# s-will/BiAlign

Hardware: AMD Instinct MI355X
Metric: giga-DP-cells/sec (higher is better)
Workload: dtype int32

## Files before the change

### bialign_amd/csrc/bialign_feed.hpp

```cpp
#pragma once

namespace bialign {

template <int S, int NL, bool LEAN = false, int BLKO = 0>
struct GhostFeed {
  using R_ = Rec<S, NL, LEAN>;
  static constexpr int W = 2 * S + 1, R = 64 / W;
  static constexpr int NP = R_::NCH4 + (R_::TAIL ? 1 : 0);
#ifdef BIALIGN_BLK_OVERRIDE
  static constexpr int BLK = BIALIGN_BLK_OVERRIDE;
#else
  static constexpr int BLK = BLKO ? BLKO : (S <= 1 ? 8 : 4);
#endif
  static constexpr int NPIECE = BLK * W * NP;
  static constexpr bool PIECE_MAJOR = S >= 2;
  __host__ __device__ static constexpr int slot(int t, int aa, int c) {
    return PIECE_MAJOR ? (c * BLK + t) * W + aa : (t * W + aa) * NP + c;
  }
  static constexpr int ROUNDS = (NPIECE + 63) / 64;
  static constexpr int SLOTS = ROUNDS * 64;
  static constexpr int RING_DW = 2 * SLOTS * 4;
  static constexpr int MIN_GOFF = 2 * BLK + 8;

  __device__ static __forceinline__ void issue(const int32_t* lay, int h0, int blk_q, int blk_rem,
                                               int P, int T, int w, int GOFF, int rec_last, int lane,
                                               uint32_t lds_base) {
#pragma unroll
    for (int r = 0; r < ROUNDS; ++r) {
      const int q = min(r * 64 + lane, NPIECE - 1);
      int t, aa, c;
      if (PIECE_MAJOR) {
        c = q / (BLK * W);
        const int rem = q - c * (BLK * W);
        t = rem / W;
        aa = rem - t * W;
      } else {
        t = q / (W * NP);
        const int rem = q - t * (W * NP);
        aa = rem / NP;
        c = rem - aa * NP;
      }
      const int xr = blk_rem + t - aa;
      const int ql = blk_q + (xr >= P ? 1 : 0) - (xr < 0 ? 1 : 0);
      const int rec = min(max(h0 + t - GOFF + (ql * (T - 1) + w) * P, 0), rec_last);
      const int sl = LEAN ? aa : (R - 2) * W + aa;
      const int32_t* p = lay + (int64_t)rec * R_::RECDW +
                         (c < R_::NCH4 ? c * R_::CH + sl * 4 : R_::NCH4 * R_::CH + sl * R_::TAIL);
      const uint32_t dst = lds_base + r * 1024;
      uint32_t keep;
      asm volatile(
          "s_mov_b32 %0, m0\n\ts_mov_b32 m0, %2\n\ts_nop 0\n\t"
          "global_load_lds_dwordx4 %1, off sc1\n\ts_mov_b32 m0, %0"
          : "=&s"(keep)
          : "v"(p), "s"(dst)
          : "memory");
    }
  }
  __host__ __device__ static inline void piece_of(int q, int& t, int& aa, int& c) {
    if (PIECE_MAJOR) {
      c = q / (BLK * W);
      const int rem = q - c * (BLK * W);
      t = rem / W;
      aa = rem - t * W;
    } else {
      t = q / (W * NP);
      const int rem = q - t * (W * NP);
      aa = rem / NP;
      c = rem - aa * NP;
    }
  }
  __host__ __device__ static inline int packed_piece_dw(int c, int sl) {
    using PK = Pack<S>;
    return c < PK::NCH ? c * R_::CH + sl * 4 : (c == PK::NCH && PK::TAILDW ? PK::NCH * R_::CH + sl * PK::TAILDW : sl * 4);
  }
  template <typename Base>
  __host__ __device__ static inline Base packed_src(Base lay, int q, int64_t bnd_off, int blk_q, int blk_rem, int P, int T,
                                                    int w, int m, int rec_last) {
    using PK = Pack<S>;
    int t, aa, c;
    piece_of(q, t, aa, c);
    const int xr = blk_rem + t - aa;
    const int ql = blk_q + (xr >= P ? 1 : 0) - (xr < 0 ? 1 : 0);
    const int jj = xr - (xr >= P ? P : 0) + (xr < 0 ? P : 0);
    const int ts = jj + 2 * (R - 1) + aa;
    const int cs = ts >= P ? ts - P : ts, qs = ql * T + w - 1 + (ts >= P ? 1 : 0);
    const int64_t rec = (int64_t)(ql * T + w - 1) * P + ts;
    const bool valid = rec >= 0 && rec <= rec_last;
    const int sl = (R - 2) * W + aa;
    if (valid && PK::interior(qs, cs, m)) return lay + rec * PK::RECDW + packed_piece_dw(c, sl);
    return lay + bnd_off + (valid ? PK::bidx(qs, cs, P, m) : 0) * R_::RECDW +
           (c < R_::NCH4 ? c * R_::CH + sl * 4 : R_::NCH4 * R_::CH + sl * R_::TAIL);
  }
  __device__ static __forceinline__ void issue_packed(const int32_t* lay, int64_t bnd_off, int m, int h0, int blk_q,
                                                      int blk_rem, int P, int T, int w, int rec_last, int lane,
                                                      uint32_t lds_base) {
#pragma unroll
    for (int r = 0; r < ROUNDS; ++r) {
      const int q = min(r * 64 + lane, NPIECE - 1);
      const int32_t* p = packed_src(lay, q, bnd_off, blk_q, blk_rem, P, T, w, m, rec_last);
      const uint32_t dst = lds_base + r * 1024;
      uint32_t keep;
      asm volatile(
          "s_mov_b32 %0, m0\n\ts_mov_b32 m0, %2\n\ts_nop 0\n\t"
          "global_load_lds_dwordx4 %1, off sc1\n\ts_mov_b32 m0, %0"
          : "=&s"(keep)
          : "v"(p), "s"(dst)
          : "memory");
    }
  }

  __host__ __device__ static inline bool steady(int blk_q, int blk_rem, int P, int T, int w, int m, int rec_last) {
    using PK = Pack<S>;
    const int qs = blk_q * T + w - 1, ts_last = blk_rem + BLK - 1 + 2 * (R - 1);
    return qs >= PK::Q0 && blk_rem >= 3 * S + 1 && ts_last <= m - S && (int64_t)qs * P + ts_last <= rec_last;
  }
  __host__ __device__ static inline int64_t steady_base_dword(int blk_q, int blk_rem, int P, int T, int w) {
    return ((int64_t)(blk_q * T + w - 1) * P + blk_rem + 2 * (R - 1)) * Pack<S>::RECDW;
  }
  __host__ __device__ static inline uint32_t lane_offset(int r, int lane) {
    int t, aa, c;
    piece_of(r * 64 + lane < NPIECE - 1 ? r * 64 + lane : NPIECE - 1, t, aa, c);
    return (uint32_t)(t * Pack<S>::RECDW + packed_piece_dw(c, (R - 2) * W + aa)) * 4u;
  }
  static constexpr int OFFTAB_DW = ROUNDS * 64;
  __device__ static __forceinline__ void issue_steady(const int32_t* lay, int blk_q, int blk_rem, int P, int T, int w,
                                                      const int32_t* offtab, int lane, uint32_t lds_base) {
    const int32_t* base = lay + steady_base_dword(blk_q, blk_rem, P, T, w);
    uint32_t off[ROUNDS];
#pragma unroll
    for (int r = 0; r < ROUNDS; ++r) off[r] = (uint32_t)offtab[r * 64 + lane];
#pragma unroll
    for (int r = 0; r < ROUNDS; ++r) {
      const uint32_t dst = lds_base + r * 1024;
      uint32_t keep;
      asm volatile(
          "s_mov_b32 %0, m0\n\ts_mov_b32 m0, %2\n\ts_nop 0\n\t"
          "global_load_lds_dwordx4 %1, %3 sc1\n\ts_mov_b32 m0, %0"
          : "=&s"(keep)
          : "v"(off[r]), "s"(dst), "s"(base)
          : "memory");
    }
  }
  static constexpr int STORES_PER_STEP = R_::NCH4 + (R_::TAIL ? 1 : 0);

  __device__ static __forceinline__ void wait_block(int younger) {
    if (younger > 40) asm volatile("s_waitcnt vmcnt(40)" ::: "memory");
    else if (younger > 24) asm volatile("s_waitcnt vmcnt(24)" ::: "memory");
    else if (younger > 20) asm volatile("s_waitcnt vmcnt(20)" ::: "memory");
    else if (younger > 16) asm volatile("s_waitcnt vmcnt(16)" ::: "memory");
    else if (younger > 12) asm volatile("s_waitcnt vmcnt(12)" ::: "memory");
    else if (younger > 6) asm volatile("s_waitcnt vmcnt(6)" ::: "memory");
    else if (younger > 3) asm volatile("s_waitcnt vmcnt(3)" ::: "memory");
    else if (younger > 1) asm volatile("s_waitcnt vmcnt(1)" ::: "memory");
    else asm volatile("s_waitcnt vmcnt(0)" ::: "memory");
  }

  template <int NPK>
  __device__ static __forceinline__ void fetch_pieces(int (&out)[4 * NPK], const v4i* half, int t, int aa) {
#pragma unroll
    for (int c = 0; c < NPK; ++c) {
      const v4i v = half[slot(t, aa, c)];
      out[4 * c] = v.x; out[4 * c + 1] = v.y; out[4 * c + 2] = v.z; out[4 * c + 3] = v.w;
    }
  }

  __device__ static __forceinline__ void fetch(int (&out)[R_::ND], const v4i* half, int t, int aa) {
#pragma unroll
    for (int c = 0; c < NP; ++c) {
      const v4i v = half[slot(t, aa, c)];
      if (4 * c + 0 < R_::ND) out[4 * c + 0 < R_::ND ? 4 * c + 0 : 0] = v.x;
      if (4 * c + 1 < R_::ND) out[4 * c + 1 < R_::ND ? 4 * c + 1 : 0] = v.y;
      if (4 * c + 2 < R_::ND) out[4 * c + 2 < R_::ND ? 4 * c + 2 : 0] = v.z;
      if (4 * c + 3 < R_::ND) out[4 * c + 3 < R_::ND ? 4 * c + 3 : 0] = v.w;
    }
  }
};

template <int S, bool LEAN>
struct GhostSrc {
  using GF = GhostFeed<S, 9, LEAN, 0>;
  static constexpr int W = 2 * S + 1, R = 64 / W;
  static constexpr int STEPB = W * GF::NP * 16;
  static constexpr int HALFB = GF::SLOTS * 16;
  __host__ __device__ static inline uint32_t ring_step_byte(int g) {
    return (uint32_t)(((g / GF::BLK) & 1) * HALFB + (g & (GF::BLK - 1)) * STEPB);
  }
  __host__ __device__ static inline uint32_t factor(int lane) { return lane < R * W ? 1u : 0u; }
  __host__ __device__ static inline uint32_t lane_byte(int lane, uint32_t sent) {
    return lane < R * W ? (uint32_t)((lane % W) * GF::NP * 16) : sent;
  }
};

template <int S>
constexpr int slim_offtab_dw() { return GhostFeed<S, 9>::OFFTAB_DW; }

template <int S>
struct Mu2Feed {
  static constexpr int BLK = GhostFeed<S, 9>::BLK;
  static constexpr int RING_DW = 2 * BLK * 64;
  __device__ static __forceinline__ void issue(const int32_t* tab, int n, int m, int P, int jj0,
                                               int strip, int T, int w, int il, int aa,
                                               uint32_t lds_base) {
    constexpr int RR = Geo<S>::RR;
#pragma unroll
    for (int t = 0; t < BLK; ++t) {
      int jf = jj0 + t, q = strip;
      if (jf >= P) { jf -= P; ++q; }
      int l = jf + S;
      if (l > m) { l = jf - P + S; ++q; }
      const int k = (q * T + w) * RR + il - 1 + aa - S;
      const int kc = min(max(k, 1), n), lc = min(max(l, 1), m);
      const int32_t* p = tab + (int64_t)(kc - 1) * m + (lc - 1);
      const uint32_t dst = lds_base + t * 256;
      uint32_t keep;
      asm volatile(
          "s_mov_b32 %0, m0\n\ts_mov_b32 m0, %2\n\ts_nop 0\n\t"
          "global_load_lds_dword %1, off\n\ts_mov_b32 m0, %0"
          : "=&s"(keep)
          : "v"(p), "s"(dst)
          : "memory");
    }
  }
};

template <int S>
struct Mu1Feed {
  static constexpr int BLK = GhostFeed<S, 9>::BLK;
  static constexpr int RING_DW = 2 * BLK * 64;
  __device__ static __forceinline__ void issue(const int32_t* tab, int n, int m, int P, int jj0, int strip,
                                               int T, int w, int il, uint32_t lds_base) {
    constexpr int RR = Geo<S>::RR;
#pragma unroll
    for (int t = 0; t < BLK; ++t) {
      int jf = jj0 + t, q = strip;
      if (jf >= P) { jf -= P; ++q; }
      const int i = (q * T + w) * RR + il - 1;
      const int ic = min(max(i, 1), n), jc = min(max(jf, 1), m);
      const int32_t* p = tab + (int64_t)(ic - 1) * m + (jc - 1);
      const uint32_t dst = lds_base + t * 256;
      uint32_t keep;
      asm volatile(
          "s_mov_b32 %0, m0\n\ts_mov_b32 m0, %2\n\ts_nop 0\n\t"
          "global_load_lds_dword %1, off\n\ts_mov_b32 m0, %0"
          : "=&s"(keep)
          : "v"(p), "s"(dst)
          : "memory");
    }
  }
};

}
```

### bialign_amd/csrc/bialign_fill_slim.hpp

```cpp
#pragma once

namespace bialign {

template <int S, int TW, int PPW, bool LEAN = false>
__global__ void __launch_bounds__(64 * TW * PPW, 3) fill_affine_slim_kernel(const DeviceBatch A) {
  static_assert(S >= 1, "packed records need a band");
  using PK_ = Pack<S>;
  using G_ = Geo<S>;
  using R_ = Rec<S, 9, LEAN>;
  constexpr int W = G_::W, R = G_::R, RR = G_::RR, PADB = G_::PADB;
  constexpr int ND = R_::ND, NCH4 = R_::NCH4, TAIL = R_::TAIL, RECDW = R_::RECDW;
  static_assert(R * W < 64, "lane 63 must be free: it is the sentinel source of the exchange");
  extern __shared__ __align__(16) int32_t smem[];

  constexpr int T = TW;
  constexpr int NW = TW * PPW;
  const int L = threadIdx.x & 63;
  const int wv = NW == 1 ? 0 : __builtin_amdgcn_readfirstlane(threadIdx.x >> 6);
  const int pw = wv / TW, w = wv - pw * TW;
  const int slot = blockIdx.x * PPW + pw;
  const bool have_pair = slot < A.launch_pairs;
  const int pid = A.order[have_pair ? slot : 0];
  const PairDesc pd = A.pairs[pid];
  const int n = pd.n, m = pd.m, P = pd.P;
  const int il = L / W, aa = L - il * W;
  const bool live = L < R * W;
  const bool ghost = (il == 0);
  int ringfed_v = (ghost || !live) ? 1 : 0;
  asm volatile("" : "+v"(ringfed_v));
  const bool ringfed = ringfed_v != 0;
  int storing_v;
  {
    const int pad_idx0 = L < W ? L : (L >= R * W ? W + (L - R * W) : 64);
    storing_v = ((live && (LEAN ? il == R - 1 : !ghost)) || (!LEAN && pad_idx0 < R_::SLP - R_::SL)) ? 1 : 0;
  }
  asm volatile("" : "+v"(storing_v));
  const bool storing = storing_v != 0;
  const int beta = A.beta, gamma = A.gamma, delta = A.delta;
  const int k1 = A.k1, k2 = A.k2;
  const int gD = gamma + delta, gg = 2 * gamma, ggdd = 2 * gamma + 2 * delta, dd = 2 * delta;

  using GF = GhostFeed<S, 9, LEAN, 0>;
  constexpr int PERW = GF::RING_DW;
  constexpr int SENTBLK = 4 * GF::NP;
  v4i* ring = reinterpret_cast<v4i*>(smem + wv * GF::RING_DW);
  int32_t* sentblk = smem + NW * PERW;
  volatile int32_t* prog_lds = smem + NW * PERW + SENTBLK + pw * TW;
  const volatile int32_t* const fit_floor = smem + NW * PERW + SENTBLK + FIT_FLOOR_WORD;
  const volatile int32_t* const col0_floor = smem + NW * PERW + SENTBLK + COL0_FLOOR_WORD;
  int32_t* offtab = smem + NW * PERW + SENTBLK + LDS_PROG_WORDS;
  int32_t* s1 = offtab + slim_offtab_dw<S>();
  int32_t* s2 = s1 + k1 * k1;
  uint8_t* codes = reinterpret_cast<uint8_t*>(s2 + k2 * k2);
  const int npad = code_pad(n), mpad = code_pad(m, PADB);
  uint8_t* sa = codes + (size_t)pw * A.slim_code_bytes;
  uint8_t* ca = sa + npad;
  uint8_t* sb = ca + npad;
  uint8_t* cb = sb + mpad;

  for (int t = threadIdx.x; t < NW * PERW + SENTBLK; t += 64 * NW) smem[t] = SENT;
  if (threadIdx.x < LDS_PROG_WORDS) smem[NW * PERW + SENTBLK + threadIdx.x] = prog_word_init(threadIdx.x, A.fit);
  if (!LEAN)
    for (int t = threadIdx.x; t < GF::OFFTAB_DW; t += 64 * NW) offtab[t] = (int32_t)GF::lane_offset(t >> 6, t & 63);
  for (int t = threadIdx.x; t < k1 * k1; t += 64 * NW) s1[t] = A.s1[t];
  for (int t = threadIdx.x; t < k2 * k2; t += 64 * NW) s2[t] = A.s2[t];
  if (have_pair) {
    const int tt = threadIdx.x - pw * (64 * TW);
    for (int t = tt; t < n; t += 64 * TW) {
      sa[t] = A.seq_a[pd.seq_a + t];
      ca[t] = A.cls_a[pd.seq_a + t];
    }
    for (int t = tt; t < m + 2 * PADB; t += 64 * TW) {
      const int src = t - PADB;
      const bool ok = src >= 0 && src < m;
      sb[t] = ok ? A.seq_b[pd.seq_b + src] : 0;
      cb[t] = ok ? A.cls_b[pd.seq_b + src] : 0;
    }
  }
  __syncthreads();
  if (!have_pair) return;

  const int addrA = ((L - W) & 63) * 4;
  const int addrB = (live && aa < W - 1 ? ((L - W + 1) & 63) : 63) * 4;
  const bool a_first = (aa == 0);
  const int lane_cap = a_first ? SENT : 0x7fffffff;
  int32_t* const lay = A.layers + pd.layer_off;
  const int64_t pk_bnd_off = (int64_t)pd.G * PK_::RECDW;
  const int rec_last = pd.G - 1;
  const int NSw = (pd.NS - w + T - 1) / T;
  const int H = NSw > 0 ? (NSw - 1) * P + m + G_::MAXOFF + 1 : 0;

  int jj = -(2 * il + aa);
  int strip = 0;
  int rec_base = w * P;
  int i = 0, s1row = 0, s2row = 0;
  bool act_row = false;
  auto set_row = [&](int q) {
    i = (q * T + w) * RR + il - 1;
    const int k = i + aa - S;
    act_row = live && i >= 0 && i <= n && k >= 0 && k <= n;
    s1row = (i >= 1 && i <= n) ? sa[i - 1] * k1 : 0;
    s2row = (k >= 1 && k <= n) ? ca[k - 1] * k2 : 0;
  };
  set_row(0);

  int dA1[2][W], dA2[2][W];
  int dAx[2][W];
  int dB[4][W];
  int dC[2][W];
  int selfv[4][W];
  int pubC[W][8];
  int inC[W][8];
  int inA[W][4], inB[W][8];
#pragma unroll
  for (int bb = 0; bb < W; ++bb) {
    dA1[0][bb] = dA1[1][bb] = dA2[0][bb] = dA2[1][bb] = SENT;
    dAx[0][bb] = dAx[1][bb] = dC[0][bb] = dC[1][bb] = SENT;
#pragma unroll
    for (int x = 0; x < 4; ++x) dB[x][bb] = selfv[x][bb] = inA[bb][x] = SENT;
#pragma unroll
    for (int x = 0; x < 8; ++x) pubC[bb][x] = inB[bb][x] = inC[bb][x] = SENT;
  }
  const uint32_t ring_lds = __builtin_amdgcn_readfirstlane(
      (uint32_t)(uintptr_t)(__attribute__((address_space(3))) int32_t*)smem) + wv * GF::RING_DW * 4;

  using SA = StepAddr<S, LEAN>;
  using GS = GhostSrc<S, LEAN>;
  typedef const __attribute__((address_space(3))) int32_t* lds_cptr;
  typedef __attribute__((address_space(1))) char* gbl_ptr;
  typedef __attribute__((address_space(1))) v4i* gbl_v4i;
  typedef __attribute__((address_space(1))) int32_t* gbl_i32;
  uint32_t st_off = SA::chunk_off(L), st_toff = SA::tail_off(L), gs_fac = GS::factor(L);
  uint32_t gs_lane = GS::lane_byte(L, ring_lds + (NW - wv) * GF::RING_DW * 4);
  asm volatile("" : "+v"(st_off), "+v"(st_toff), "+v"(gs_fac), "+v"(gs_lane));
  int s_ph = 0, s_q = 0;
  int s_adv = 0;
  uint32_t ring_u = 0;
  gbl_ptr sbase = nullptr;

  int blk_q = 0, blk_rem = 0;
  int seen_prog = -0x40000000;
  auto wait_partner = [&](int h_last) __attribute__((always_inline)) {
    if (T == 1) return;
    const int src = w == 0 ? T - 1 : w - 1;
    const int need = h_last + 2 * (R - 1) + 1 - (w == 0 ? P : 0);
    if (seen_prog >= need) return;
    for (int spin = 0; (seen_prog = prog_lds[src]) < need; ++spin) {
      if (spin > A.spin_limit) {
        if (L == 0) atomicOr(A.errflag, 1);
        seen_prog = 0x7fffffff;
        break;
      }
      __builtin_amdgcn_s_sleep(16);
    }
  };
  bool blk_steady = false;
  auto prefetch_block = [&](int h0, int half) __attribute__((always_inline)) {
    wait_partner(h0 + GF::BLK - 1);
    if (!LEAN) blk_steady = GF::steady(blk_q, blk_rem, P, T, w, m, rec_last);
    int Lv = L;
    asm volatile("" : "+v"(Lv));
    if (!LEAN && blk_steady)
      GF::issue_steady(lay, blk_q, blk_rem, P, T, w, offtab, Lv, ring_lds + half * GF::SLOTS * 16);
    else if (LEAN) GF::issue(lay, h0, blk_q, blk_rem, P, T, w, P - 2 * (R - 1), rec_last, Lv, ring_lds + half * GF::SLOTS * 16);
    else GF::issue_packed(lay, pk_bnd_off, m, h0, blk_q, blk_rem, P, T, w, rec_last, Lv, ring_lds + half * GF::SLOTS * 16);
    blk_rem += GF::BLK;
    if (blk_rem >= P) { blk_rem -= P; ++blk_q; }
  };
  prefetch_block(0, 0);
  asm volatile("s_waitcnt vmcnt(0)" ::: "memory");
  int vm_younger = 0;
  int pk_all = 0;
  static_assert(LEAN || PK_::check_in_every_gap(GF::BLK),
                "range check: a test must fall into every non-interior stretch between two strips (pk_all is cleared, not kept, once a row leaves the lattice)");

  auto dmov = [](int& dst, int src) __attribute__((always_inline)) { asm("v_mov_b32 %0, %1" : "=v"(dst) : "v"(src)); };
  auto bperm = [](int addr, int v) __attribute__((always_inline)) -> int { return __builtin_amdgcn_ds_bpermute(addr, v); };

  int mu1n = 0, mu2n[W], sbn = 0, cbn = 0;
  auto lookup_mu = [&]() __attribute__((always_inline)) {
    const int jc = min(max(jj, 0), m + 1);
    mu1n = s1[s1row + sb[jc - 1 + PADB]];
#pragma unroll
    for (int bb = 0; bb < W; ++bb) mu2n[bb] = s2[s2row + cb[jc + bb]];
  };
  auto fetch_codes = [&](auto clamp_tag) __attribute__((always_inline)) {
    const int jc1 = decltype(clamp_tag)::value ? min(max(jj + 1, 0), m + 1) : jj + s_adv + 1;
    sbn = sb[jc1 - 1 + PADB];
    cbn = cb[jc1 + W - 1];
  };
  lookup_mu();
  fetch_codes(BoolTag<true>{});
  int fit_best = SENT, fit_j = 0;

  auto step = [&](auto interior_tag, int g) __attribute__((always_inline)) {
    constexpr bool INTERIOR = decltype(interior_tag)::value;
    if (!INTERIOR) {
      jj += s_adv;
      s_adv = 0;
    }
    const int gt = g & (GF::BLK - 1), ghalf = (g / GF::BLK) & 1;
    if (gt == 0) {
      GF::wait_block(vm_younger);
      if (TW > 1 && L == 0) prog_lds[w] = g - GF::BLK;
      if (!LEAN && (g & (PK_::CHECK - 1)) == 0) {
        const bool bad = live && !ghost && (unsigned)pk_all > 0xffffu;
        if (__builtin_amdgcn_ballot_w64(bad) != 0 && L == 0) atomicOr(A.errflag, 2);
        pk_all = 0;
      }
      if (!LEAN) {
        if (L < GF::BLK * W) {
          bool packed = true;
          if (!blk_steady) {
            int ph = s_ph + L / W, qst = s_q * T + w;
            if (ph >= P) { ph -= P; qst += T; }
            const int ts = ph + 2 * (R - 1), over = ts >= P ? 1 : 0;
            packed = PK_::interior(qst - 1 + over, ts - over * P, m);
          }
          if (packed) {
            v4i* pc = ring + ghalf * GF::SLOTS + L * GF::NP;
            int raw[4 * PK_::NPC], dec[4 * GF::NP];
#pragma unroll
            for (int c = 0; c < PK_::NPC; ++c) {
              const v4i v = pc[c];
              raw[4 * c] = v.x; raw[4 * c + 1] = v.y; raw[4 * c + 2] = v.z; raw[4 * c + 3] = v.w;
            }
#pragma unroll
            for (int d = 0; d < 4 * GF::NP; ++d) {
              const int h = PK_::hw(d < ND ? d : 0);
              const unsigned word = (unsigned)raw[d < ND && d != PK_::ANCHOR ? h >> 1 : 0];
              const unsigned e = d == PK_::ANCHOR ? 0x8000u : PK_::offset_of((h & 1) ? word >> 16 : word & 0xffffu, raw[0]);
              const int v = raw[0] + (int)e;
              dec[d] = d >= ND ? 0 : (pack_corner(W, d % 9, d / 9) ? (e == 0xffffu ? NEG : v) : v);
            }
#pragma unroll
            for (int c = 0; c < GF::NP; ++c) {
              v4i v;
              v.x = dec[4 * c]; v.y = dec[4 * c + 1]; v.z = dec[4 * c + 2]; v.w = dec[4 * c + 3];
              pc[c] = v;
            }
          }
        }
      }
      prefetch_block(g + GF::BLK, ghalf ^ 1);
      vm_younger = 0;
      ring_u = ring_lds + ghalf * GS::HALFB;
      if (A.prio_mode) {
        const int lvl = ((g >> 7) + (wv >> 2)) & 3;
        if (lvl == 0) __builtin_amdgcn_s_setprio(0);
        else if (lvl == 1) __builtin_amdgcn_s_setprio(1);
        else if (lvl == 2) __builtin_amdgcn_s_setprio(2);
        else __builtin_amdgcn_s_setprio(3);
      }
    }
    const int32_t* const gsrc = live ? reinterpret_cast<const int32_t*>(ring + ghalf * GF::SLOTS + (gt * W + aa) * GF::NP)
                                     : sentblk;
    uint32_t gaddr = 0;
    if (INTERIOR) asm("v_mad_u32_u24 %0, %1, %2, %3" : "=v"(gaddr) : "v"(gs_fac), "s"(ring_u), "v"(gs_lane));
    const lds_cptr gsrc_s = (lds_cptr)(uintptr_t)gaddr;
    auto at_store = [](uint32_t& off) __attribute__((always_inline)) -> uint32_t {
      asm volatile("" : "+v"(off));
      return off;
    };

    auto read_dpp = [&](int r) __attribute__((always_inline)) { dpp_from_left<W>(r, inC, pubC, lane_cap); };
    read_dpp(0);

    const int mu1 = mu1n;
    int mu2[W];
#pragma unroll
    for (int bb = 0; bb < W; ++bb) mu2[bb] = mu2n[bb];

    const bool tile_act = INTERIOR ? true : (act_row && jj >= 0 && jj <= m);
    const bool is_origin = INTERIOR ? false : (tile_act && i == 0 && jj == 0 && aa == S);
    const bool row0_diag = INTERIOR ? false : (tile_act && i == 0 && aa == S);
    const bool col0_diag = INTERIOR ? false : (tile_act && jj == 0 && aa == S);
    const int c3M = mu1 + dd, c_Mg = mu1 + gD;

    const int rec = g + rec_base;
    const int pad_idx = L < W ? L : (L >= R * W ? W + (L - R * W) : 64);
    const bool pad_lane = pad_idx < R_::SLP - R_::SL;
    constexpr bool PACKED = INTERIOR && !LEAN;
    const bool do_store = INTERIOR ? storing
                                   : (((live && (LEAN ? il == R - 1 : !ghost)) || (!LEAN && pad_lane)) &&
                                      __builtin_amdgcn_ballot_w64(tile_act && !ghost) != 0 && (TW == 1 || rec <= rec_last));
    const int slot_ = LEAN ? aa : (pad_lane ? R_::SL + pad_idx : L - W);
    if (INTERIOR) vm_younger += PACKED ? PK_::NPC : GF::STORES_PER_STEP;
    else if (__builtin_amdgcn_ballot_w64(do_store) != 0) vm_younger += GF::STORES_PER_STEP;
    int32_t* dst = lay + (int64_t)rec * RECDW;
    if (!INTERIOR && !LEAN) {
      const int tl = jj + 2 * il + aa;
      const int over = tl >= P ? 1 : 0;
      dst = lay + pk_bnd_off + PK_::bidx(strip * T + w + over, tl - over * P, P, m) * RECDW;
    }

    int outv[PACKED ? 1 : ND];
    int pk_base = 0, pk_min = 0, pk_max = 0, pk_e[PACKED ? ND : 1];
    int h2y[3] = {SENT, SENT, SENT};
    int defer[3] = {SENT, SENT, SENT};
#pragma unroll
    for (int bb = 0; bb < W; ++bb) {
      if (bb + 1 < W) read_dpp(bb + 1 < W ? bb + 1 : 0);
      const int l = jj + bb - S;
      const bool act = INTERIOR ? true : (tile_act && l >= 0 && l <= m);
      const int mu2v = mu2[bb];
      const int c_MM = mu1 + mu2v, c_gM = mu2v + gD, c2M = mu2v + dd;

      const AffineCases<W> cases{dA2, bb, dB, dAx, inB, dC, selfv, c_MM, c_Mg, c_gM, gg, ggdd, inC, h2y, c2M, gD, c3M};
      int M[9];
      bool isneg[9] = {};
      if (INTERIOR) {
        if (ringfed) {
#pragma unroll
          for (int q = 0; q < 9; ++q) M[q] = gsrc_s[bb * 9 + q];
        } else {
          int Tv[9];
          cases(Tv);
#pragma unroll
          for (int q = 0; q < 9; ++q) {
            int tv = Tv[q];
            if (can_be_empty<W>(q / 3, q % 3, bb)) {
              isneg[q] = tv < THRESH;
              tv = isneg[q] ? NEG : tv;
            }
            M[q] = tv;
          }
        }
      } else {
        int Gm[9];
#pragma unroll
        for (int q = 0; q < 9; ++q) Gm[q] = SENT;
        if (ghost) {
#pragma unroll
          for (int q = 0; q < 9; ++q) Gm[q] = gsrc[bb * 9 + q];
        }
        int Tv[9];
        cases(Tv);
        const int low = act ? NEG : SENT;
#pragma unroll
        for (int q = 0; q < 9; ++q) {
          const int tv = ghost ? Gm[q] : Tv[q];
          const bool bad = (tv < THRESH) | !act;
          M[q] = bad ? low : tv;
        }
        if (bb == S) M[8] = is_origin ? 0 : M[8];
        if (bb == S && row0_diag) M[8] = imax(M[8], fit_floor[0]);
        if (bb == S && col0_diag) M[8] = imax(M[8], col0_floor[0]);
      }
      if (!PACKED) {
#pragma unroll
        for (int q = 0; q < 9; ++q) outv[PACKED ? 0 : bb * 9 + q] = M[q];
      }
      if (LEAN && bb == S) {
        if (!INTERIOR && live && !ghost && aa == S && i == n && jj == m && !A.fit) {
          int best = M[0];
#pragma unroll
          for (int q = 1; q < 9; ++q) best = imax(best, M[q]);
          A.scores[pid] = best;
        }
        if (A.fit) {
          const int col = INTERIOR ? jj + s_adv : jj;
          if (live && !ghost && aa == S && i == n && (INTERIOR || (col >= 0 && col <= m))) {
            int best = M[0];
#pragma unroll
            for (int q = 1; q < 9; ++q) best = imax(best, M[q]);
            if (best > fit_best) fit_best = best, fit_j = col;
            if (!INTERIOR && col == m) {
              if (A.fit & FREE_A_ENDS) {
                atomicMax(A.local_key + pid, local_key_of(fit_best, n, fit_j, m));
              } else {
                A.scores[pid] = fit_best;
                A.fit_span[2 * pid + 1] = fit_j;
              }
            }
          } else if (!INTERIOR && (A.fit & FREE_A_ENDS) && live && !ghost && aa == S && act_row && col == m) {
            int best = M[0];
#pragma unroll
            for (int q = 1; q < 9; ++q) best = imax(best, M[q]);
            atomicMax(A.local_key + pid, local_key_of(best, i, m, m));
          }
        }
      }
      if (PACKED) {
        if (bb == 0) {
          pk_base = M[8] - 0x8000;
          pk_min = pk_max = M[8];
        }
        {
          int xs[9];
          int nx = 0;
#pragma unroll
          for (int q = 0; q < 9; ++q) {
            if (bb * 9 + q == PK_::ANCHOR) continue;
            int x = M[q];
            if (pack_corner(W, q, bb)) {
              const bool ng = isneg[q];
              x = ng ? pk_base + 0xffff : x;
            }
            pk_e[PACKED ? bb * 9 + q : 0] = x;
            xs[nx++] = x;
          }
#pragma unroll
          for (int t = 0; t + 1 < nx; t += 2) pk_min = imin(imin(pk_min, xs[t]), xs[t + 1]);
          if (nx & 1) pk_min = imin(pk_min, xs[nx - 1]);
        }
        if (do_store) {
#pragma unroll
          for (int c = 0; c < PK_::NPC; ++c) {
            constexpr int NDWc = PK_::NDW;
            const int dlast = 4 * c + 3 < NDWc - 1 ? 4 * c + 3 : NDWc - 1;
            const int last = PK_::val(2 * dlast + 1);
            if (last >= bb * 9 && last < (bb + 1) * 9) {
              int dw[4];
#pragma unroll
              for (int x = 0; x < 4; ++x) {
                const int d = 4 * c + x;
                const int lo = d < NDWc ? PK_::val(2 * d) : 0, hi = d < NDWc ? PK_::val(2 * d + 1) : 0;
                dw[x] = d == 0 ? pk_base
                               : (d < NDWc ? (int)__builtin_amdgcn_perm((unsigned)pk_e[PACKED ? hi : 0], (unsigned)pk_e[PACKED ? lo : 0], 0x05040100u) : 0);
              }
              if (c < PK_::NCH) {
                v4i v;
                v.x = dw[0]; v.y = dw[1]; v.z = dw[2]; v.w = dw[3];
                *reinterpret_cast<gbl_v4i>(sbase + SA::chunk_imm(c) + at_store(st_off)) = v;
              } else if (slot_ < PK_::TSLOTS) {
                const gbl_i32 tp = reinterpret_cast<gbl_i32>(sbase + SA::TAIL_IMM + at_store(st_toff));
#pragma unroll
                for (int x = 0; x < PK_::TAILDW; ++x) tp[x] = dw[x];
              }
            }
          }
        }
      } else {
        if (do_store) {
#pragma unroll
          for (int c = 0; c < NCH4; ++c) {
            if (4 * c + 3 >= bb * 9 && 4 * c + 3 < (bb + 1) * 9) {
              v4i v;
              v.x = outv[PACKED ? 0 : 4 * c]; v.y = outv[PACKED ? 0 : 4 * c + 1];
              v.z = outv[PACKED ? 0 : 4 * c + 2]; v.w = outv[PACKED ? 0 : 4 * c + 3];
              if (INTERIOR) *reinterpret_cast<gbl_v4i>(sbase + SA::chunk_imm(c) + at_store(st_off)) = v;
              else *reinterpret_cast<v4i*>(dst + c * R_::CH + slot_ * 4) = v;
            }
          }
          if (LEAN && bb == W - 1) {
            const gbl_i32 tp = INTERIOR ? reinterpret_cast<gbl_i32>(sbase + SA::TAIL_IMM + at_store(st_toff)) : nullptr;
#pragma unroll
            for (int t = 0; t < TAIL; ++t) {
              if (INTERIOR) tp[t] = outv[PACKED ? 0 : 4 * NCH4 + t];
              else dst[NCH4 * R_::CH + slot_ * TAIL + t] = outv[PACKED ? 0 : 4 * NCH4 + t];
            }
          }
        }
        if (!LEAN && bb == W - 1) {
          const bool wave_stores = __builtin_amdgcn_ballot_w64(tile_act && !ghost) != 0 && (TW == 1 || rec <= rec_last);
          if (wave_stores) {
            const int tslot = (live && !ghost) ? L - W : R_::SL + (L < W ? L : W + (L - R * W));
#pragma unroll
            for (int t = 0; t < TAIL; ++t) dst[NCH4 * R_::CH + tslot * TAIL + t] = outv[PACKED ? 0 : 4 * NCH4 + t];
          }
        }
      }

      int H2[3][3], H3[3][3], Gd[3][3];
#pragma unroll
      for (int u = 0; u < 3; ++u) {
        H2[u][2] = fM(M[3 * u], M[3 * u + 1], M[3 * u + 2]);
        const int bm = beta + H2[u][2];
        H2[u][0] = imax(M[3 * u], bm);
        H2[u][1] = imax(M[3 * u + 1], bm);
      }
#pragma unroll
      for (int v = 0; v < 3; ++v) {
        H3[2][v] = fM(M[v], M[3 + v], M[6 + v]);
        Gd[2][v] = fM(H2[0][v], H2[1][v], H2[2][v]);
        const int bm3 = beta + H3[2][v], bmg = beta + Gd[2][v];
        H3[0][v] = imax(M[v], bm3);
        H3[1][v] = imax(M[3 + v], bm3);
        Gd[0][v] = imax(H2[0][v], bmg);
        Gd[1][v] = imax(H2[1][v], bmg);
      }
      if (PACKED) {
        pk_max = imax(pk_max, Gd[2][2]);
        if (bb == W - 1) {
          const int acc = pk_all | (pk_max - pk_base + 1) | (pk_min - pk_base);
          pk_all = act_row ? acc : 0;
        }
      }
      pubC[bb][0] = Gd[0][2];
      pubC[bb][1] = Gd[0][1];
#pragma unroll
      for (int u = 0; u < 3; ++u) {
        pubC[bb][2 + u] = H2[u][2];
        pubC[bb][5 + u] = H2[u][1];
      }
      selfv[0][bb] = Gd[0][0];
#pragma unroll
      for (int v = 0; v < 3; ++v) selfv[1 + v][bb] = H3[0][v];
#pragma unroll
      for (int u = 0; u < 3; ++u) h2y[u] = H2[u][0];

      dmov(dA2[0][bb], dA1[0][bb]);
      dmov(dA2[1][bb], dA1[1][bb]);
      dmov(dA1[0][bb], inA[bb][0]);
      dmov(dA1[1][bb], inA[bb][1]);
      dmov(dB[0][bb], inB[bb][0]);
#pragma unroll
      for (int v = 0; v < 3; ++v) dmov(dB[1 + v][bb], inB[bb][2 + v]);
      dC[0][bb] = inC[bb][0];
      dC[1][bb] = inC[bb][1];
      inA[bb][0] = bperm(addrA, Gd[2][2]);
      inA[bb][1] = bperm(addrA, Gd[2][1]);
      inB[bb][0] = bperm(addrB, Gd[2][0]);
#pragma unroll
      for (int v = 0; v < 3; ++v) {
        inB[bb][2 + v] = bperm(addrB, H3[2][v]);
        inB[bb][5 + v] = bperm(addrB, H3[1][v]);
      }
      if (bb >= 1) {
        dmov(dAx[0][bb >= 1 ? bb - 1 : 0], inA[bb >= 1 ? bb - 1 : 0][2]);
        dmov(dAx[1][bb >= 1 ? bb - 1 : 0], inA[bb >= 1 ? bb - 1 : 0][3]);
        inA[bb >= 1 ? bb - 1 : 0][2] = bperm(addrA, defer[0]);
        inA[bb >= 1 ? bb - 1 : 0][3] = bperm(addrA, defer[1]);
        inB[bb >= 1 ? bb - 1 : 0][1] = bperm(addrB, defer[2]);
      }
      defer[0] = Gd[1][2];
      defer[1] = Gd[1][1];
      defer[2] = Gd[1][0];
    }
    dmov(dAx[0][W - 1], inA[W - 1][2]);
    dmov(dAx[1][W - 1], inA[W - 1][3]);
    inA[W - 1][2] = bperm(addrA, defer[0]);
    inA[W - 1][3] = bperm(addrA, defer[1]);
    inB[W - 1][1] = bperm(addrB, defer[2]);

    if (INTERIOR) ++s_adv;
    else ++jj;
    if (!INTERIOR && jj == P) {
      jj = 0;
      ++strip;
      rec_base += (T - 1) * P;
      set_row(strip);
    }
    ++s_ph;
    if (!INTERIOR && s_ph == P) {
      s_ph = 0;
      ++s_q;
    }
    ring_u += GS::STEPB;
    if (INTERIOR) {
      sbase += SA::RECB;
    } else {
      const uint64_t b = (uint64_t)(uintptr_t)(reinterpret_cast<char*>(lay) + SA::record_byte(g + 1, s_q, T, w, P));
      sbase = reinterpret_cast<gbl_ptr>((uintptr_t)((uint64_t)__builtin_amdgcn_readfirstlane((uint32_t)(b >> 32)) << 32 |
                                                    (uint32_t)__builtin_amdgcn_readfirstlane((uint32_t)b)));
    }
    if (INTERIOR) {
      mu1n = s1[s1row + sbn];
#pragma unroll
      for (int bb = 0; bb + 1 < W; ++bb) dmov(mu2n[bb], mu2[bb + 1]);
      mu2n[W - 1] = s2[s2row + cbn];
    } else {
      lookup_mu();
    }
    if (INTERIOR) fetch_codes(BoolTag<false>{});
    else fetch_codes(BoolTag<true>{});
  };

  auto all_interior = [&]() __attribute__((always_inline)) {
    (void)jj, (void)strip;
    return PK_::interior(s_q * T + w, s_ph, m);
  };
  int g = 0;
  while (g < H) {
    while (g < H && !all_interior()) {
      step(BoolTag<false>{}, g);
      ++g;
    }
    while (g < H && all_interior()) {
      step(BoolTag<true>{}, g);
      ++g;
    }
  }
  if (!LEAN && __builtin_amdgcn_ballot_w64(live && !ghost && (unsigned)pk_all > 0xffffu) != 0 && L == 0) atomicOr(A.errflag, 2);
  if (TW > 1) {
    asm volatile("s_waitcnt vmcnt(0)" ::: "memory");
    if (L == 0) prog_lds[w] = 0x7fffffff;
  }
}

}
```

Measured before the change: 210.5.

## Streamline boundary-step addressing, ghost feed and steady prefetch in slim fill kernel

Carries the steady-prefetch record index incrementally and issues the three LDS-direct loads in one asm block that bumps m0. Boundary steps now use wave-uniform scalar base pointers (bnd0/bnd1, sbase minus an offset) instead of per-lane bidx address math. Ghost lanes read directly from the LDS ring via the shared mad address, and the threshold masking is simplified. The vmcnt wait ladder is coarsened and setprio is only touched every 128 steps. The goal is fewer VALU/SALU instructions per DP step. The risks are coarser waits that stall longer and subtle boundary-address correctness.

```diff
diff --git a/bialign_amd/csrc/bialign_feed.hpp b/bialign_amd/csrc/bialign_feed.hpp
--- a/bialign_amd/csrc/bialign_feed.hpp
+++ b/bialign_amd/csrc/bialign_feed.hpp
@@ -122,13 +122,31 @@
     piece_of(r * 64 + lane < NPIECE - 1 ? r * 64 + lane : NPIECE - 1, t, aa, c);
     return (uint32_t)(t * Pack<S>::RECDW + packed_piece_dw(c, (R - 2) * W + aa)) * 4u;
   }
+  __host__ __device__ static inline int steady_rec(int blk_q, int blk_rem, int P, int T, int w) {
+    return (blk_q * T + w - 1) * P + blk_rem + 2 * (R - 1);
+  }
+  __host__ __device__ static inline bool steady_carried(int qs, int blk_rem, int rec0, int m, int rec_last) {
+    return qs >= Pack<S>::Q0 && blk_rem >= 3 * S + 1 && blk_rem + BLK - 1 + 2 * (R - 1) <= m - S && rec0 + BLK - 1 <= rec_last;
+  }
   static constexpr int OFFTAB_DW = ROUNDS * 64;
-  __device__ static __forceinline__ void issue_steady(const int32_t* lay, int blk_q, int blk_rem, int P, int T, int w,
-                                                      const int32_t* offtab, int lane, uint32_t lds_base) {
-    const int32_t* base = lay + steady_base_dword(blk_q, blk_rem, P, T, w);
+  __device__ static __forceinline__ void issue_steady(const int32_t* base, const int32_t* offtab, int lane, uint32_t lds_base) {
     uint32_t off[ROUNDS];
 #pragma unroll
     for (int r = 0; r < ROUNDS; ++r) off[r] = (uint32_t)offtab[r * 64 + lane];
+    if (ROUNDS == 3) {
+      uint32_t keep;
+      asm volatile(
+          "s_mov_b32 %0, m0\n\ts_mov_b32 m0, %4\n\ts_nop 0\n\t"
+          "global_load_lds_dwordx4 %1, %5 sc1\n\t"
+          "s_add_u32 m0, m0, 0x400\n\ts_nop 0\n\t"
+          "global_load_lds_dwordx4 %2, %5 sc1\n\t"
+          "s_add_u32 m0, m0, 0x400\n\ts_nop 0\n\t"
+          "global_load_lds_dwordx4 %3, %5 sc1\n\ts_mov_b32 m0, %0"
+          : "=&s"(keep)
+          : "v"(off[0]), "v"(off[ROUNDS > 1 ? 1 : 0]), "v"(off[ROUNDS > 2 ? 2 : 0]), "s"(lds_base), "s"(base)
+          : "memory", "scc");
+      return;
+    }
 #pragma unroll
     for (int r = 0; r < ROUNDS; ++r) {
       const uint32_t dst = lds_base + r * 1024;
@@ -155,6 +173,14 @@
     else asm volatile("s_waitcnt vmcnt(0)" ::: "memory");
   }
 
+  __device__ static __forceinline__ void wait_block_slim(int younger) {
+    if (younger > 40) asm volatile("s_waitcnt vmcnt(40)" ::: "memory");
+    else if (younger > 24) asm volatile("s_waitcnt vmcnt(24)" ::: "memory");
+    else if (younger > 12) asm volatile("s_waitcnt vmcnt(12)" ::: "memory");
+    else if (younger > 3) asm volatile("s_waitcnt vmcnt(3)" ::: "memory");
+    else asm volatile("s_waitcnt vmcnt(0)" ::: "memory");
+  }
+
   template <int NPK>
   __device__ static __forceinline__ void fetch_pieces(int (&out)[4 * NPK], const v4i* half, int t, int aa) {
 #pragma unroll
diff --git a/bialign_amd/csrc/bialign_fill_slim.hpp b/bialign_amd/csrc/bialign_fill_slim.hpp
--- a/bialign_amd/csrc/bialign_fill_slim.hpp
+++ b/bialign_amd/csrc/bialign_fill_slim.hpp
@@ -44,7 +44,6 @@
   constexpr int PERW = GF::RING_DW;
   constexpr int SENTBLK = 4 * GF::NP;
   v4i* ring = reinterpret_cast<v4i*>(smem + wv * GF::RING_DW);
-  int32_t* sentblk = smem + NW * PERW;
   volatile int32_t* prog_lds = smem + NW * PERW + SENTBLK + pw * TW;
   const volatile int32_t* const fit_floor = smem + NW * PERW + SENTBLK + FIT_FLOOR_WORD;
   const volatile int32_t* const col0_floor = smem + NW * PERW + SENTBLK + COL0_FLOOR_WORD;
@@ -136,9 +135,20 @@
   int s_ph = 0, s_q = 0;
   int s_adv = 0;
   uint32_t ring_u = 0;
-  gbl_ptr sbase = nullptr;
+  auto uniform_ptr = [](uint64_t b) __attribute__((always_inline)) -> gbl_ptr {
+    return reinterpret_cast<gbl_ptr>((uintptr_t)((uint64_t)__builtin_amdgcn_readfirstlane((uint32_t)(b >> 32)) << 32 |
+                                                 (uint32_t)__builtin_amdgcn_readfirstlane((uint32_t)b)));
+  };
+  gbl_ptr sbase = uniform_ptr((uint64_t)(uintptr_t)(reinterpret_cast<char*>(lay) + SA::record_byte(0, 0, T, w, P)));
+  constexpr int FULLB = R_::RECDW * 4;
+  auto bnd_record = [&](int qs) __attribute__((always_inline)) -> gbl_ptr {
+    return uniform_ptr((uint64_t)(uintptr_t)(reinterpret_cast<char*>(lay + pk_bnd_off) + PK_::bidx(qs, 0, P, m) * FULLB));
+  };
+  gbl_ptr bnd0 = LEAN ? nullptr : bnd_record(w), bnd1 = bnd0;
+  const int64_t lean_back = (int64_t)(T - 1) * P * FULLB;
 
   int blk_q = 0, blk_rem = 0;
+  int blk_rec = GF::steady_rec(0, 0, P, T, w);
   int seen_prog = -0x40000000;
   auto wait_partner = [&](int h_last) __attribute__((always_inline)) {
     if (T == 1) return;
@@ -157,15 +167,16 @@
   bool blk_steady = false;
   auto prefetch_block = [&](int h0, int half) __attribute__((always_inline)) {
     wait_partner(h0 + GF::BLK - 1);
-    if (!LEAN) blk_steady = GF::steady(blk_q, blk_rem, P, T, w, m, rec_last);
+    if (!LEAN) blk_steady = GF::steady_carried(blk_q * T + w - 1, blk_rem, blk_rec, m, rec_last);
     int Lv = L;
     asm volatile("" : "+v"(Lv));
     if (!LEAN && blk_steady)
-      GF::issue_steady(lay, blk_q, blk_rem, P, T, w, offtab, Lv, ring_lds + half * GF::SLOTS * 16);
+      GF::issue_steady(lay + (int64_t)blk_rec * PK_::RECDW, offtab, Lv, ring_lds + half * GF::SLOTS * 16);
     else if (LEAN) GF::issue(lay, h0, blk_q, blk_rem, P, T, w, P - 2 * (R - 1), rec_last, Lv, ring_lds + half * GF::SLOTS * 16);
     else GF::issue_packed(lay, pk_bnd_off, m, h0, blk_q, blk_rem, P, T, w, rec_last, Lv, ring_lds + half * GF::SLOTS * 16);
     blk_rem += GF::BLK;
-    if (blk_rem >= P) { blk_rem -= P; ++blk_q; }
+    blk_rec += GF::BLK;
+    if (blk_rem >= P) { blk_rem -= P; ++blk_q; blk_rec += (T - 1) * P; }
   };
   prefetch_block(0, 0);
   asm volatile("s_waitcnt vmcnt(0)" ::: "memory");
@@ -201,7 +212,7 @@
     }
     const int gt = g & (GF::BLK - 1), ghalf = (g / GF::BLK) & 1;
     if (gt == 0) {
-      GF::wait_block(vm_younger);
+      GF::wait_block_slim(vm_younger);
       if (TW > 1 && L == 0) prog_lds[w] = g - GF::BLK;
       if (!LEAN && (g & (PK_::CHECK - 1)) == 0) {
         const bool bad = live && !ghost && (unsigned)pk_all > 0xffffu;
@@ -245,7 +256,7 @@
       prefetch_block(g + GF::BLK, ghalf ^ 1);
       vm_younger = 0;
       ring_u = ring_lds + ghalf * GS::HALFB;
-      if (A.prio_mode) {
+      if (A.prio_mode && __builtin_expect((g & 127) == 0, 0)) {
         const int lvl = ((g >> 7) + (wv >> 2)) & 3;
         if (lvl == 0) __builtin_amdgcn_s_setprio(0);
         else if (lvl == 1) __builtin_amdgcn_s_setprio(1);
@@ -253,10 +264,8 @@
         else __builtin_amdgcn_s_setprio(3);
       }
     }
-    const int32_t* const gsrc = live ? reinterpret_cast<const int32_t*>(ring + ghalf * GF::SLOTS + (gt * W + aa) * GF::NP)
-                                     : sentblk;
     uint32_t gaddr = 0;
-    if (INTERIOR) asm("v_mad_u32_u24 %0, %1, %2, %3" : "=v"(gaddr) : "v"(gs_fac), "s"(ring_u), "v"(gs_lane));
+    asm("v_mad_u32_u24 %0, %1, %2, %3" : "=v"(gaddr) : "v"(gs_fac), "s"(ring_u), "v"(gs_lane));
     const lds_cptr gsrc_s = (lds_cptr)(uintptr_t)gaddr;
     auto at_store = [](uint32_t& off) __attribute__((always_inline)) -> uint32_t {
       asm volatile("" : "+v"(off));
@@ -271,28 +280,25 @@
 #pragma unroll
     for (int bb = 0; bb < W; ++bb) mu2[bb] = mu2n[bb];
 
-    const bool tile_act = INTERIOR ? true : (act_row && jj >= 0 && jj <= m);
+    const bool tile_act = INTERIOR ? true : (act_row && (unsigned)jj <= (unsigned)m);
     const bool is_origin = INTERIOR ? false : (tile_act && i == 0 && jj == 0 && aa == S);
     const bool row0_diag = INTERIOR ? false : (tile_act && i == 0 && aa == S);
     const bool col0_diag = INTERIOR ? false : (tile_act && jj == 0 && aa == S);
     const int c3M = mu1 + dd, c_Mg = mu1 + gD;
+    int neg_v = NEG;
+    if (!INTERIOR) asm volatile("" : "+v"(neg_v));
 
     const int rec = g + rec_base;
     const int pad_idx = L < W ? L : (L >= R * W ? W + (L - R * W) : 64);
     const bool pad_lane = pad_idx < R_::SLP - R_::SL;
     constexpr bool PACKED = INTERIOR && !LEAN;
-    const bool do_store = INTERIOR ? storing
-                                   : (((live && (LEAN ? il == R - 1 : !ghost)) || (!LEAN && pad_lane)) &&
-                                      __builtin_amdgcn_ballot_w64(tile_act && !ghost) != 0 && (TW == 1 || rec <= rec_last));
+    const bool wave_stores = INTERIOR ? true : (__builtin_amdgcn_ballot_w64(tile_act && !ringfed) != 0 && (TW == 1 || rec <= rec_last));
+    const bool do_store = INTERIOR ? storing : (storing && wave_stores);
     const int slot_ = LEAN ? aa : (pad_lane ? R_::SL + pad_idx : L - W);
     if (INTERIOR) vm_younger += PACKED ? PK_::NPC : GF::STORES_PER_STEP;
     else if (__builtin_amdgcn_ballot_w64(do_store) != 0) vm_younger += GF::STORES_PER_STEP;
-    int32_t* dst = lay + (int64_t)rec * RECDW;
-    if (!INTERIOR && !LEAN) {
-      const int tl = jj + 2 * il + aa;
-      const int over = tl >= P ? 1 : 0;
-      dst = lay + pk_bnd_off + PK_::bidx(strip * T + w + over, tl - over * P, P, m) * RECDW;
-    }
+    gbl_ptr dstp = nullptr;
+    if (!INTERIOR) dstp = strip == s_q ? (LEAN ? sbase : bnd0) : (LEAN ? sbase - lean_back : bnd1);
 
     int outv[PACKED ? 1 : ND];
     int pk_base = 0, pk_min = 0, pk_max = 0, pk_e[PACKED ? ND : 1];
@@ -302,7 +308,7 @@
     for (int bb = 0; bb < W; ++bb) {
       if (bb + 1 < W) read_dpp(bb + 1 < W ? bb + 1 : 0);
       const int l = jj + bb - S;
-      const bool act = INTERIOR ? true : (tile_act && l >= 0 && l <= m);
+      const bool act = INTERIOR || bb == S ? tile_act : (tile_act && (unsigned)l <= (unsigned)m);
       const int mu2v = mu2[bb];
       const int c_MM = mu1 + mu2v, c_gM = mu2v + gD, c2M = mu2v + dd;
 
@@ -327,21 +333,20 @@
           }
         }
       } else {
-        int Gm[9];
-#pragma unroll
-        for (int q = 0; q < 9; ++q) Gm[q] = SENT;
-        if (ghost) {
-#pragma unroll
-          for (int q = 0; q < 9; ++q) Gm[q] = gsrc[bb * 9 + q];
-        }
-        int Tv[9];
-        cases(Tv);
-        const int low = act ? NEG : SENT;
-#pragma unroll
-        for (int q = 0; q < 9; ++q) {
-          const int tv = ghost ? Gm[q] : Tv[q];
-          const bool bad = (tv < THRESH) | !act;
-          M[q] = bad ? low : tv;
+        if (ringfed) {
+#pragma unroll
+          for (int q = 0; q < 9; ++q) {
+            const int gv = gsrc_s[bb * 9 + q];
+            M[q] = act ? gv : SENT;
+          }
+        } else {
+          int Tv[9];
+          cases(Tv);
+          int low = act ? neg_v : SENT;
+          int bar = act ? THRESH - 1 : 0x7fffffff;
+          asm volatile("" : "+v"(low), "+v"(bar));
+#pragma unroll
+          for (int q = 0; q < 9; ++q) M[q] = Tv[q] <= bar ? low : Tv[q];
         }
         if (bb == S) M[8] = is_origin ? 0 : M[8];
         if (bb == S && row0_diag) M[8] = imax(M[8], fit_floor[0]);
@@ -440,24 +445,22 @@
               v.x = outv[PACKED ? 0 : 4 * c]; v.y = outv[PACKED ? 0 : 4 * c + 1];
               v.z = outv[PACKED ? 0 : 4 * c + 2]; v.w = outv[PACKED ? 0 : 4 * c + 3];
               if (INTERIOR) *reinterpret_cast<gbl_v4i>(sbase + SA::chunk_imm(c) + at_store(st_off)) = v;
-              else *reinterpret_cast<v4i*>(dst + c * R_::CH + slot_ * 4) = v;
+              else *reinterpret_cast<gbl_v4i>(dstp + SA::chunk_imm(c) + st_off) = v;
             }
           }
           if (LEAN && bb == W - 1) {
-            const gbl_i32 tp = INTERIOR ? reinterpret_cast<gbl_i32>(sbase + SA::TAIL_IMM + at_store(st_toff)) : nullptr;
-#pragma unroll
-            for (int t = 0; t < TAIL; ++t) {
-              if (INTERIOR) tp[t] = outv[PACKED ? 0 : 4 * NCH4 + t];
-              else dst[NCH4 * R_::CH + slot_ * TAIL + t] = outv[PACKED ? 0 : 4 * NCH4 + t];
-            }
+            const gbl_i32 tp = INTERIOR ? reinterpret_cast<gbl_i32>(sbase + SA::TAIL_IMM + at_store(st_toff))
+                                        : reinterpret_cast<gbl_i32>(dstp + SA::TAIL_IMM + st_toff);
+#pragma unroll
+            for (int t = 0; t < TAIL; ++t) tp[t] = outv[PACKED ? 0 : 4 * NCH4 + t];
           }
         }
         if (!LEAN && bb == W - 1) {
-          const bool wave_stores = __builtin_amdgcn_ballot_w64(tile_act && !ghost) != 0 && (TW == 1 || rec <= rec_last);
           if (wave_stores) {
             const int tslot = (live && !ghost) ? L - W : R_::SL + (L < W ? L : W + (L - R * W));
-#pragma unroll
-            for (int t = 0; t < TAIL; ++t) dst[NCH4 * R_::CH + tslot * TAIL + t] = outv[PACKED ? 0 : 4 * NCH4 + t];
+            const gbl_i32 tp = reinterpret_cast<gbl_i32>(dstp + NCH4 * R_::CH * 4 + tslot * (TAIL * 4));
+#pragma unroll
+            for (int t = 0; t < TAIL; ++t) tp[t] = outv[PACKED ? 0 : 4 * NCH4 + t];
           }
         }
       }
@@ -543,17 +546,23 @@
       set_row(strip);
     }
     ++s_ph;
-    if (!INTERIOR && s_ph == P) {
+    if (!INTERIOR && !LEAN) {
+      bnd0 += FULLB;
+      bnd1 += FULLB;
+    }
+    if (!INTERIOR && __builtin_expect(s_ph == P, 0)) {
       s_ph = 0;
       ++s_q;
+      if (!LEAN) {
+        bnd0 = bnd_record(s_q * T + w);
+        bnd1 = bnd_record((s_q - 1) * T + w + 1);
+      }
     }
     ring_u += GS::STEPB;
     if (INTERIOR) {
       sbase += SA::RECB;
     } else {
-      const uint64_t b = (uint64_t)(uintptr_t)(reinterpret_cast<char*>(lay) + SA::record_byte(g + 1, s_q, T, w, P));
-      sbase = reinterpret_cast<gbl_ptr>((uintptr_t)((uint64_t)__builtin_amdgcn_readfirstlane((uint32_t)(b >> 32)) << 32 |
-                                                    (uint32_t)__builtin_amdgcn_readfirstlane((uint32_t)b)));
+      sbase = uniform_ptr((uint64_t)(uintptr_t)(reinterpret_cast<char*>(lay) + SA::record_byte(g + 1, s_q, T, w, P)));
     }
     if (INTERIOR) {
       mu1n = s1[s1row + sbn];
```

Result: no change. 211.0 (median of 6 runs) (+0.2%).
